# Adttil/crypto12381

Measured on AMD Instinct MI355X. Metric: G1 scalar-muls/s per MI355X (batch 2^20 per GPU), bit-exact vs CPU, higher is better.
Workload: dtype int64 accumulate over 14x28-bit signed limbs

## Files before the change

crypto12381_amd/csrc/g1.hpp:

```cpp
#pragma once
#include "fp.hpp"

namespace c12381 {

struct g1p { fp x, y, z; };

C12381_HD void g1_set_inf(g1p& p) { fp_zero(p.x); fp_one(p.y); fp_zero(p.z); }
C12381_HD bool g1_is_inf(const g1p& p) { return fp_is_zero(p.z); }
C12381_HD void g1_norm1(g1p& r, const g1p& p) { fp_norm1(r.x, p.x); fp_norm1(r.y, p.y); fp_norm1(r.z, p.z); }
C12381_HD void g1_norm1(g1p& p) { g1_norm1(p, p); }
C12381_HD void g1_select(g1p& r, bool c, const g1p& a, const g1p& b) { fp_select(r.x, c, a.x, b.x); fp_select(r.y, c, a.y, b.y); fp_select(r.z, c, a.z, b.z); }
C12381_HD void g1_set_invalid(g1p& p) { fp_one(p.x); fp_zero(p.y); fp_zero(p.z); }
C12381_HD bool g1_is_invalid(const g1p& p) { return fp_is_zero(p.z) && !fp_is_zero(p.x); }

C12381_HD void g1_dbl(g1p& p) {
    fp t0, t1, t2, z8, u, y3, x3, z3;
    const int32_t cm3 = fp_opaque_const(-3);
    fp_mul(t1, p.y, p.z);
    fp_sqr(t2, p.z);
    fp_mul_small(t2, t2, 12);
    fp_sqr_inj(u, p.y, [&](int i, int64_t& acc) { fp_inj(acc, t2, i, cm3); }, C12381_BV(3 * t2.vb), C12381_BV(3 * t2.lb));
    fp_dbl(t0, t2); fp_add(t0, t0, t2); fp_add(t0, t0, u);
    fp_mul_small(z8, t0, 8);
    fp_add(y3, t0, t2);
// ... 163 lines not shown
    {
        uint64_t bw = 0;
#pragma unroll
        for (int i = 0; i < 5; ++i) {
            const uint64_t t = (uint64_t)k[i] - qd[i] - bw;
            rem[i] = (uint32_t)t;
            bw = (t >> 32) & 1;
        }
    }
#pragma unroll
    for (int round = 0; round < 2; ++round) {
        uint32_t d[5];
        uint64_t bw = 0;
#pragma unroll
        for (int i = 0; i < 5; ++i) {
            const uint64_t t = (uint64_t)rem[i] - (i < 4 ? GLV_X2[i] : 0u) - bw;
            d[i] = (uint32_t)t;
            bw = (t >> 32) & 1;
        }
        const bool ge = bw == 0;
#pragma unroll
        for (int i = 0; i < 5; ++i) rem[i] = ge ? d[i] : rem[i];
        uint64_t c = ge ? 1u : 0u;
#pragma unroll
        for (int i = 0; i < 4; ++i) { c += q[i]; q[i] = (uint32_t)c; c >>= 32; }
    }
#pragma unroll
    for (int i = 0; i < 4; ++i) { k0[i] = rem[i]; k1[i] = q[i]; }
}

C12381_HD void soa_store_fp(int32_t* base, size_t stride, size_t idx, const fp& a) {
#pragma unroll
    for (int i = 0; i < NL; ++i) base[(size_t)i * stride + idx] = a.l[i];
}
C12381_HD void soa_load_fp(fp& a, const int32_t* base, size_t stride, size_t idx) {
#pragma unroll
    for (int i = 0; i < NL; ++i) a.l[i] = base[(size_t)i * stride + idx];
    C12381_BOUNDS(a.lb = 268435456.0 + 8.0; a.vb = 4.0; check_actual(a, "soa_load_fp");)
}
C12381_HD void soa_store_g1(int32_t* base, size_t stride, size_t idx, const g1p& p) {
    soa_store_fp(base, stride, idx, p.x);
    soa_store_fp(base + (size_t)NL * stride, stride, idx, p.y);
    soa_store_fp(base + (size_t)2 * NL * stride, stride, idx, p.z);
}
C12381_HD void soa_load_g1(g1p& p, const int32_t* base, size_t stride, size_t idx) {
    soa_load_fp(p.x, base, stride, idx);
    soa_load_fp(p.y, base + (size_t)NL * stride, stride, idx);
    soa_load_fp(p.z, base + (size_t)2 * NL * stride, stride, idx);
}

constexpr int G1_WIN = 5;
constexpr int G1_TAB = 1 << (G1_WIN - 1);
constexpr int G1_WINDOWS = 26;
constexpr int G1_ENT_DWORDS = 44;
constexpr int G1_TAB_DWORDS = G1_TAB * G1_ENT_DWORDS;
struct alignas(16) q4 { int32_t v[4]; };
struct alignas(8) d2 { int32_t v[2]; };

template <int Q0, int NQ, class P>
C12381_HD void rec_store_q4(P dst, const int32_t* w) {
#pragma unroll
    for (int i = Q0; i < Q0 + NQ; ++i) { q4 t; t.v[0] = w[4 * i]; t.v[1] = w[4 * i + 1]; t.v[2] = w[4 * i + 2]; t.v[3] = w[4 * i + 3]; dst[i] = t; }
}
template <int Q0, int NQ, class P>
C12381_HD void rec_load_q4(int32_t* w, P src) {
#pragma unroll
    for (int i = Q0; i < Q0 + NQ; ++i) { q4 t = src[i]; w[4 * i] = t.v[0]; w[4 * i + 1] = t.v[1]; w[4 * i + 2] = t.v[2]; w[4 * i + 3] = t.v[3]; }
}

constexpr double G1_REC_LB = 268435456.0 + 8.0;
template <bool KEEP_PADS = false>
C12381_HD void tab_store_fields(int32_t* ent, const fp& a, const fp& b, const fp& c) {
    int32_t w[G1_ENT_DWORDS];
#pragma unroll
    for (int i = 0; i < NL; ++i) { w[i] = a.l[i]; w[NL + i] = b.l[i]; w[2 * NL + i] = c.l[i]; }
    w[42] = 0; w[43] = 0;
    rec_store_q4<0, G1_ENT_DWORDS / 4 - (KEEP_PADS ? 1 : 0)>(reinterpret_cast<q4*>(ent), w);
    if (KEEP_PADS) { d2 t; t.v[0] = w[40]; t.v[1] = w[41]; *reinterpret_cast<d2*>(ent + 40) = t; }
}
template <bool KEEP_PADS = false>
C12381_HD void tab_store_rec(int32_t* ent, const fp& a, const fp& b, const fp& c, double vb_cap) {
    (void)vb_cap;
    C12381_BOUNDS(for (const fp* e : {&a, &b, &c}) { if (e->vb > vb_cap) bounds_fail("tab_store_rec value bound", e->vb, vb_cap);
                                                      if (e->lb > G1_REC_LB) bounds_fail("tab_store_rec limb bound", e->lb, G1_REC_LB); })
    tab_store_fields<KEEP_PADS>(ent, a, b, c);
}
template <int Q0, int NQ>
C12381_HD void tab_load_q4(int32_t (&w)[G1_ENT_DWORDS], const int32_t* ent) { rec_load_q4<Q0, NQ>(w, reinterpret_cast<const q4*>(ent)); }
C12381_HD void rec_field(fp& a, const int32_t (&w)[G1_ENT_DWORDS], int off, double vb_cap) {
#pragma unroll
    for (int i = 0; i < NL; ++i) a.l[i] = w[off + i];
    (void)vb_cap;
    C12381_BOUNDS(a.lb = G1_REC_LB; a.vb = vb_cap; check_actual(a, "rec_field");)
}
C12381_HD void tab_load_rec(fp& a, fp& b, fp& c, const int32_t* ent, double vb_cap) {
    int32_t w[G1_ENT_DWORDS];
    tab_load_q4<0, G1_ENT_DWORDS / 4>(w, ent);
    rec_field(a, w, 0, vb_cap); rec_field(b, w, NL, vb_cap); rec_field(c, w, 2 * NL, vb_cap);
}
C12381_HD void tab_store_g1(int32_t* ent, const g1p& p) { tab_store_fields(ent, p.x, p.y, p.z); }
C12381_HD void tab_load_g1(g1p& p, const int32_t* ent) { tab_load_rec(p.x, p.y, p.z, ent, 4.0); }

constexpr uint32_t glv_bias_word5(int i) {
    uint32_t v = 0;
    for (int w = 0; w < 26; ++w) { const int bit = 5 * w + 4; if ((bit >> 5) == i) v |= 1u << (bit & 31); }
    return v;
}
C12381_HD int glv_digit(const uint32_t (&kb)[5], int w) {
    const int bit = 5 * w, word = bit >> 5, sh = bit & 31;
    uint32_t v = kb[word] >> sh;
    if (sh > 27) v |= kb[word + 1] << (32 - sh);
    return (int)(v & 31u) - 16;
}
C12381_HD void glv_bias(uint32_t (&kb)[5], const uint32_t (&k)[4]) {
    constexpr uint32_t B[5] = {glv_bias_word5(0), glv_bias_word5(1), glv_bias_word5(2), glv_bias_word5(3), glv_bias_word5(4)};
    uint64_t c = 0;
#pragma unroll
    for (int i = 0; i < 4; ++i) { c += (uint64_t)k[i] + B[i]; kb[i] = (uint32_t)c; c >>= 32; }
    kb[4] = (uint32_t)c + B[4];
}
C12381_HD void glv_scalar_digits(uint32_t (&kb0)[5], uint32_t (&kb1)[5], const uint32_t (&kin)[8], bool zero = false) {
    uint32_t k[8], k0[4], k1[4];
#pragma unroll
    for (int i = 0; i < 8; ++i) k[i] = kin[i];
    scalar_mod_r(k);
    scalar_glv_split(k0, k1, k);
#pragma unroll
    for (int i = 0; i < 4; ++i) { k0[i] = zero ? 0u : k0[i]; k1[i] = zero ? 0u : k1[i]; }
    glv_bias(kb0, k0);
    glv_bias(kb1, k1);
}
C12381_HD const int32_t* g1_digit_entry(const int32_t* lane_tab, int d) {
    const int mag = d < 0 ? -d : d;
    return lane_tab + ((mag == 0 ? 1 : mag) - 1) * G1_ENT_DWORDS;
}
C12381_HD void g1_sched_fence() {
#if defined(__HIP_DEVICE_COMPILE__)
    __builtin_amdgcn_sched_barrier(0);
#endif
}
C12381_HD void g1_digit_fix(g1p& r, g1p q, int d, bool endo);
C12381_HD void g1_digit_point(g1p& r, const int32_t* lane_tab, int d, bool endo) {
    g1p q;
    tab_load_g1(q, g1_digit_entry(lane_tab, d));
    g1_digit_fix(r, q, d, endo);
}
C12381_HD void g1_digit_fix(g1p& r, g1p q, int d, bool endo) {
    const int mag = d < 0 ? -d : d;
    fp ny;
    g1p inf;
    fp_neg(ny, q.y);
    fp_select(q.y, d < 0, ny, q.y);
    g1_set_inf(inf);
    g1_select(q, mag == 0, inf, q);
    C12381_BOUNDS(q.x.lb = q.y.lb = q.z.lb = 268435456.0 + 8.0;)
    if (endo) g1_endo_x2(r, q); else r = q;
}
C12381_HD void g1_add_digit(g1p& acc, const int32_t* lane_tab, int d, bool endo) {
    g1p e;
    g1_digit_point(e, lane_tab, d, endo);
    g1_add(acc, e);
}

C12381_HDN void g1_mul_absx(g1p& p) {
    g1p base, acc;
    g1_norm1(base, p);
    acc = base;
#pragma unroll 1
    for (int i = 62; i >= 0; --i) {
        g1_dbl(acc);
        if ((BLS_X_W[i >> 5] >> (i & 31)) & 1u) g1_add(acc, base);
    }
    p = acc;
}
C12381_HDN void g1_glv_small_scalar_term(g1p& acc, const g1p& base) {
    fp beta;
    fp_set_const(beta, FP_BETA_A);
    g1p q, s1, t;
    fp_mul(q.x, base.x, beta); q.y = base.y; q.z = base.z;
    g1_norm1(q, q);
    s1 = q;
    g1_mul_absx(s1); g1_mul_absx(s1);
    g1_norm1(s1, s1);
    fp_mul(t.x, q.x, beta); t.y = q.y; t.z = q.z;
    g1_norm1(t, t);
    {
        g1p u = s1;
        g1_add(u, t);
        if (g1_is_inf(u)) return;
    }
    g1p s2 = s1;
    g1_mul_absx(s2); g1_mul_absx(s2);
    fp_neg(t.y, s1.y); t.x = s1.x; t.z = s1.z;
    g1_norm1(t, t);
    g1_add(s2, t);
    g1_norm1(s2, s2);
    g1_add(s2, q);
    g1_norm1(s2, s2);
    g1_norm1(acc, acc);
    g1_add(acc, s2);
}

C12381_HDN void g1_scalar_mul_complete(g1p& acc, const fp& px, const fp& py, bool p_is_inf, const uint32_t (&kin)[8], int32_t* lane_tab) {
    uint32_t kb0[5], kb1[5];
    glv_scalar_digits(kb0, kb1, kin);

    g1p base, t;
    base.x = px; base.y = py; fp_one(base.z);
    {
        g1p inf;
        g1_set_inf(inf);
        g1_select(base, p_is_inf, inf, base);
    }
    tab_store_g1(lane_tab, base);
    t = base;
    g1_dbl(t);
    g1_norm1(t);
    tab_store_g1(lane_tab + G1_ENT_DWORDS, t);
#pragma unroll 1
    for (int j = 3; j <= G1_TAB; ++j) {
        if ((j & 1) == 0) {
            tab_load_g1(t, lane_tab + (j / 2 - 1) * G1_ENT_DWORDS);
            g1_dbl(t);
        } else {
            g1_add(t, base);
        }
        g1_norm1(t);
        tab_store_g1(lane_tab + (j - 1) * G1_ENT_DWORDS, t);
    }

    g1_digit_point(acc, lane_tab, glv_digit(kb0, G1_WINDOWS - 1), false);
    g1_norm1(acc);
    g1_add_digit(acc, lane_tab, glv_digit(kb1, G1_WINDOWS - 1), true);
#pragma unroll 1
    for (int w = G1_WINDOWS - 2; w >= 0; --w) {
        const int d0 = glv_digit(kb0, w), d1 = glv_digit(kb1, w);
        g1p q0, q1, e;
        tab_load_g1(q0, g1_digit_entry(lane_tab, d0));
        g1_sched_fence();
#pragma unroll 1
        for (int j = 0; j < G1_WIN; ++j) g1_dbl(acc);
        tab_load_g1(q1, g1_digit_entry(lane_tab, d1));
        g1_sched_fence();
        g1_digit_fix(e, q0, d0, false);
        g1_add(acc, e);
        g1_digit_fix(e, q1, d1, true);
        g1_add(acc, e);
    }
}

C12381_HD void tab_load_xy(fp& x, fp& y, const int32_t* ent) {
    int32_t w[G1_ENT_DWORDS];
    tab_load_q4<0, 7>(w, ent);
    rec_field(x, w, 0, 4.0); rec_field(y, w, NL, 4.0);
}
C12381_HD void tab_load_ybx(fp& y, fp& bx, const int32_t* ent) {
    int32_t w[G1_ENT_DWORDS];
    tab_load_q4<3, 8>(w, ent);
    rec_field(y, w, NL, 4.0); rec_field(bx, w, 2 * NL, 4.0);
}
C12381_HD void tab_fetch_xy(fp& x, fp& y, const int32_t* lane_tab, int d) { tab_load_xy(x, y, g1_digit_entry(lane_tab, d)); g1_sched_fence(); }
C12381_HD void tab_fetch_ybx(fp& y, fp& bx, const int32_t* lane_tab, int d) { tab_load_ybx(y, bx, g1_digit_entry(lane_tab, d)); g1_sched_fence(); }
C12381_HD void tab_store_zt(int32_t* lane_tab, const fp& zt) {
#pragma unroll
    for (int j = 0; j < NL / 2; ++j) { d2 t; t.v[0] = zt.l[2 * j]; t.v[1] = zt.l[2 * j + 1]; *reinterpret_cast<d2*>(lane_tab + j * G1_ENT_DWORDS + 42) = t; }
}
C12381_HD void tab_load_zt(fp& zt, const int32_t* lane_tab) {
#pragma unroll
    for (int j = 0; j < NL / 2; ++j) { const d2 t = *reinterpret_cast<const d2*>(lane_tab + j * G1_ENT_DWORDS + 42); zt.l[2 * j] = t.v[0]; zt.l[2 * j + 1] = t.v[1]; }
    C12381_BOUNDS(zt.lb = G1_REC_LB; zt.vb = 4.0; check_actual(zt, "tab_load_zt");)
}

template <class OnH>
C12381_HD void g1_coz_forward(int32_t* lane_tab, const fp& px, const fp& py, const fp& beta, const OnH& on_h) {
    fp x1, y1, xj, yj, xn, yn, h, hn, bx;
    g1j_dblu(xj, yj, x1, y1, px, py);
#pragma unroll 1
    for (int j = 2; j < G1_TAB; ++j) {
        g1j_zaddu(xn, yn, x1, y1, h, xj, yj);
        fp_norm1(hn, h);
        tab_store_rec(lane_tab + (j - 1) * G1_ENT_DWORDS, xj, yj, hn, 32.0);
        on_h(j, hn);
        xj = xn; yj = yn;
    }
    fp_mul(bx, xj, beta);
    tab_store_rec(lane_tab + (G1_TAB - 1) * G1_ENT_DWORDS, xj, yj, bx, 4.0);
    fp_mul(bx, x1, beta);
    tab_store_rec(lane_tab, x1, y1, bx, 4.0);
}
template <bool KEEP_PADS>
C12381_HD void g1_coz_backward(int32_t* ent, fp& mu, bool first, const fp& beta) {
    fp m2, m3, x, y, h, bx;
    tab_load_rec(x, y, h, ent, 32.0);
    if (first) mu = h; else fp_mul(mu, mu, h);
    fp_sqr(m2, mu);
    fp_mul(m3, m2, mu);
    fp_mul(x, x, m2);
    fp_mul(y, y, m3);
    fp_mul(bx, x, beta);
    tab_store_rec<KEEP_PADS>(ent, x, y, bx, 4.0);
}
C12381_HD void g1j_dbl_window(g1j& a) { g1j_dbl(a); g1j_dbl(a); g1j_dbl(a); g1j_dbl(a); g1j_dbl(a); }

C12381_HD void g1j_add_digit(g1j& acc, bool& acc_inf, const fp& x, const fp& y, int d, bool endo) {
    fp ny, ys, one;
    fp_neg(ny, y);
    fp_select(ys, (d < 0) != endo, ny, y);
    g1j r;
    g1j_madd(r, acc, x, ys);
    fp_one(one);
    fp_select(r.x, acc_inf, x, r.x); fp_select(r.y, acc_inf, ys, r.y); fp_select(r.z, acc_inf, one, r.z);
    const bool keep = d == 0;
    fp_select(acc.x, keep, acc.x, r.x); fp_select(acc.y, keep, acc.y, r.y); fp_select(acc.z, keep, acc.z, r.z);
    acc_inf = acc_inf && keep;
}
C12381_HD bool g1_coz_finish(g1p& acc, const g1j& a, const fp& zc, bool inf) {
    fp z, z2;
    fp_mul(z, a.z, zc);
    const bool exc = !inf && fp_is_zero(z);
    fp_sqr(z2, z);
    fp_mul(acc.x, a.x, z);
    acc.y = a.y;
    fp_mul(acc.z, z2, z);
    g1p o;
    g1_set_inf(o);
    g1_select(acc, inf, o, acc);
    return exc;
}

C12381_HD bool g1_scalar_mul(g1p& acc, const fp& px, const fp& py, bool p_is_inf, const uint32_t (&kin)[8], int32_t* lane_tab) {
    uint32_t kb0[5], kb1[5];
    glv_scalar_digits(kb0, kb1, kin);

    fp beta;
    fp_set_const(beta, FP_BETA_A);
    g1_coz_forward(lane_tab, px, py, beta, [](int, const fp&) {});
    {
        fp mu, zt, y2;
#pragma unroll 1
        for (int j = G1_TAB - 1; j >= 2; --j) g1_coz_backward<false>(lane_tab + (j - 1) * G1_ENT_DWORDS, mu, j == G1_TAB - 1, beta);
        fp_raw_dbl(y2, py);
        fp_mul(zt, mu, y2);
        tab_store_zt(lane_tab, zt);
    }

    g1j a;
    bool acc_inf;
    {
        const int d0 = glv_digit(kb0, G1_WINDOWS - 1);
        fp x, y, ny;
        tab_load_xy(x, y, g1_digit_entry(lane_tab, d0));
        fp_neg(ny, y);
        a.x = x;
        fp_select(a.y, d0 < 0, ny, y);
        fp_one(a.z);
        acc_inf = d0 == 0;
        const int d1 = glv_digit(kb1, G1_WINDOWS - 1);
        tab_load_ybx(y, x, g1_digit_entry(lane_tab, d1));
        g1j_add_digit(a, acc_inf, x, y, d1, true);
    }
#pragma unroll 1
    for (int w = G1_WINDOWS - 2; w >= 0; --w) {
        const int d0 = glv_digit(kb0, w), d1 = glv_digit(kb1, w);
        fp x0, y0, x1, y1;
        tab_fetch_xy(x0, y0, lane_tab, d0);
        g1j_dbl_window(a);
        tab_fetch_ybx(y1, x1, lane_tab, d1);
        g1j_add_digit(a, acc_inf, x0, y0, d0, false);
        g1j_add_digit(a, acc_inf, x1, y1, d1, true);
    }

    fp zt;
    tab_load_zt(zt, lane_tab);
    const bool exc = g1_coz_finish(acc, a, zt, acc_inf || p_is_inf);
    if (exc) g1_scalar_mul_complete(acc, px, py, p_is_inf, kin, lane_tab);
    return exc;
}
C12381_HD void tab_store_kb(int32_t* lane_tab, const uint32_t (&kb0)[5], const uint32_t (&kb1)[5]) {
#pragma unroll
    for (int j = 0; j < 5; ++j) { d2 t; t.v[0] = (int32_t)kb0[j]; t.v[1] = (int32_t)kb1[j]; *reinterpret_cast<d2*>(lane_tab + (NL / 2 + j) * G1_ENT_DWORDS + 42) = t; }
}
C12381_HD void tab_load_kb(uint32_t (&kb0)[5], uint32_t (&kb1)[5], const int32_t* lane_tab) {
#pragma unroll
    for (int j = 0; j < 5; ++j) { const d2 t = *reinterpret_cast<const d2*>(lane_tab + (NL / 2 + j) * G1_ENT_DWORDS + 42); kb0[j] = (uint32_t)t.v[0]; kb1[j] = (uint32_t)t.v[1]; }
}

template <int K, class In>
C12381_HD bool g1_scalar_mul_sum(g1p& acc, const In& in, int32_t* lane_tab) {
    static_assert(K >= 1 && K <= 4, "terms per lane");
    fp beta;
    fp_set_const(beta, FP_BETA_A);
#pragma unroll 1
    for (int t = 0; t < K; ++t) {
        int32_t* tab = lane_tab + t * G1_TAB_DWORDS;
        fp px, py;
        bool p_is_inf;
        uint32_t k[8], kb0[5], kb1[5];
        in(t, px, py, p_is_inf, k);
        glv_scalar_digits(kb0, kb1, k, p_is_inf);
        fp zrun, zt, y2, one;
        g1_coz_forward(tab, px, py, beta, [&](int j, const fp& hn) { if (j == 2) zrun = hn; else fp_mul(zrun, zrun, hn); });
        fp_raw_dbl(y2, py);
        fp_mul(zt, zrun, y2);
        fp_one(one);
        fp_select(zt, p_is_inf, one, zt);
        tab_store_zt(tab, zt);
        tab_store_kb(tab, kb0, kb1);
    }
#pragma unroll 1
    for (int t = 0; t < K; ++t) {
        int32_t* tab = lane_tab + t * G1_TAB_DWORDS;
        fp mu;
        if (K > 1) {
            fp m2, m3, x, y, h, bx;
            bool first = true;
#pragma unroll 1
            for (int l = 0; l < K; ++l) {
                if (l == t) continue;
                tab_load_zt(h, lane_tab + l * G1_TAB_DWORDS);
                if (first) mu = h; else fp_mul(mu, mu, h);
                first = false;
            }
            fp_sqr(m2, mu);
            fp_mul(m3, m2, mu);
#pragma unroll 1
            for (int e = 0; e < 2; ++e) {
                int32_t* ent = tab + (e == 0 ? 0 : G1_TAB - 1) * G1_ENT_DWORDS;
                tab_load_rec(x, y, bx, ent, 4.0);
                fp_mul(x, x, m2);
                fp_mul(y, y, m3);
                fp_mul(bx, bx, m2);
                tab_store_rec<true>(ent, x, y, bx, 4.0);
            }
        }
#pragma unroll 1
        for (int j = G1_TAB - 1; j >= 2; --j) g1_coz_backward<true>(tab + (j - 1) * G1_ENT_DWORDS, mu, K == 1 && j == G1_TAB - 1, beta);
    }

    uint32_t kb[2 * K][5];
#pragma unroll
    for (int t = 0; t < K; ++t) tab_load_kb(kb[2 * t], kb[2 * t + 1], lane_tab + t * G1_TAB_DWORDS);
    g1j a;
    fp_one(a.x); a.y = a.x; a.z = a.x;
    bool acc_inf = true;
#pragma unroll 1
    for (int w = G1_WINDOWS - 1; w >= 0; --w) {
        fp x0, y0, x1, y1;
        int d0 = glv_digit(kb[0], w);
        tab_fetch_xy(x0, y0, lane_tab, d0);
        if (w < G1_WINDOWS - 1) g1j_dbl_window(a);
        const int32_t* tab = lane_tab;
#pragma unroll 1
        for (int t = 0; t < K; ++t) {
            const int d1 = glv_digit(kb[1], w);
            tab_fetch_ybx(y1, x1, tab, d1);
            g1j_add_digit(a, acc_inf, x0, y0, d0, false);
            if (K > 1) {
#pragma unroll
                for (int i = 0; i < 5; ++i) {
                    const uint32_t r0 = kb[0][i], r1 = kb[1][i];
#pragma unroll
                    for (int j = 0; j + 2 < 2 * K; ++j) kb[j][i] = kb[j + 2][i];
                    kb[2 * K - 2][i] = r0; kb[2 * K - 1][i] = r1;
                }
                tab += G1_TAB_DWORDS;
                if (t + 1 < K) {
                    d0 = glv_digit(kb[0], w);
                    tab_fetch_xy(x0, y0, tab, d0);
                }
            }
            g1j_add_digit(a, acc_inf, x1, y1, d1, true);
        }
    }

    fp zc, z;
    tab_load_zt(zc, lane_tab);
#pragma unroll 1
    for (int t = 1; t < K; ++t) {
        tab_load_zt(z, lane_tab + t * G1_TAB_DWORDS);
        fp_mul(zc, zc, z);
    }
    const bool exc = g1_coz_finish(acc, a, zc, acc_inf);
    if (exc) {
#pragma unroll 1
        for (int t = 0; t < K; ++t) {
            fp px, py;
            bool p_is_inf;
            uint32_t k[8];
            in(t, px, py, p_is_inf, k);
            g1p term, n;
            g1_scalar_mul_complete(term, px, py, p_is_inf, k, lane_tab);
            g1_norm1(n, term);
            if (t == 0) { acc = n; continue; }
            g1_add(acc, n);
            g1_norm1(acc);
        }
    }
    return exc;
}
C12381_HD bool scalar_below_x2(const uint32_t (&kin)[8]) {
    uint32_t k[8];
#pragma unroll
    for (int i = 0; i < 8; ++i) k[i] = kin[i];
    scalar_mod_r(k);
    uint64_t bw = 0;
#pragma unroll
    for (int i = 0; i < 4; ++i) { uint64_t t = (uint64_t)k[i] - GLV_X2[i] - bw; bw = (t >> 32) & 1; }
    return (k[4] | k[5] | k[6] | k[7]) == 0u && bw == 1;
}

C12381_HD void g1_to_affine(fp& ax, fp& ay, const g1p& p, const fp& zinv) {
    fp_mul(ax, p.x, zinv);
    fp_mul(ay, p.y, zinv);
}

C12381_HD bool g1_set_x(fp& y, const fp& x, int s) {
    fp x2, x3, four, rhs, c, cinv, ny;
    fp_sqr(x2, x); fp_mul(x3, x2, x);
    fp_set_const(four, FP_FOUR);
    fp_add(rhs, x3, four);
    const bool qr = fp_sqrt_progen(c, cinv, rhs);
    fp_neg(ny, c);
    fp_select(y, fp_sign(c) != s, ny, c);
    return qr;
}

}
```

crypto12381_amd/csrc/k_g1.hip:

```cpp
#include "kernels_common.hpp"
#include "msm.hpp"

using namespace c12381;

namespace c12381 {

__global__ void __launch_bounds__(BLOCK, 2) fp_op_kernel(int op, size_t n, const uint8_t* a, const uint8_t* b, uint8_t* out) {
    const size_t i = (size_t)blockIdx.x * BLOCK + threadIdx.x;
    if (i >= n) return;
    uint32_t raw[12];
    fp x, y, r;
    load_raw48(raw, a + 48 * i); fp_from_raw48(x, raw);
    if (b) { load_raw48(raw, b + 48 * i); fp_from_raw48(y, raw); } else { fp_zero(y); }
    switch (op) {
        case 0: fp_mul(r, x, y); break;
        case 1: fp_add(r, x, y); break;
        case 2: fp_sub(r, x, y); break;
        case 3: fp_sqr(r, x); break;
        case 4: fp_neg(r, x); break;
        default: fp_inv(r, x); break;
    }
    fp_to_raw48(raw, r);
    store_raw48(out + 48 * i, raw);
}

__global__ void __launch_bounds__(BLOCK, 2) fp_mulchain_kernel(size_t n, int iters, const uint8_t* a, const uint8_t* b, uint8_t* out) {
    const size_t i = (size_t)blockIdx.x * BLOCK + threadIdx.x;
    if (i >= n) return;
    uint32_t raw[12];
    fp x, y;
    load_raw48(raw, a + 48 * i); fp_from_raw48(x, raw);
    load_raw48(raw, b + 48 * i); fp_from_raw48(y, raw);
#pragma unroll 1
    for (int it = 0; it < iters; ++it) {
        fp z;
        fp_mul(z, x, y);
        x = y; y = z;
    }
    fp_to_raw48(raw, y);
    store_raw48(out + 48 * i, raw);
}

__global__ void __launch_bounds__(BLOCK, G1_OCC) g1_mul_kernel(size_t n, const uint8_t* pts, size_t pt_stride, const uint8_t* scalars, int32_t* tab,
                                                       int32_t* proj, size_t proj_stride, size_t proj_off, int* bad_flag, const int32_t* skip_if,
                                                       int small_term) {
    if (skip_if && skip_if[HDR_VALID] != 0) return;
    const size_t i = (size_t)blockIdx.x * BLOCK + threadIdx.x;
    if (i >= n) return;
    fp px, py;
    bool inf, ok;
    g1_parse_any(px, py, inf, ok, pts, pt_stride, i);
    uint32_t raw[8], k[8];
    load_raw32(raw, scalars + 32 * i);
    scalar_from_raw32(k, raw);
    g1p acc;
    g1_scalar_mul(acc, px, py, inf || !ok, k, tab + i * (size_t)G1_TAB_DWORDS);
    if (small_term && ok && !inf && scalar_below_x2(k)) {
        g1p base, nn;
        base.x = px; base.y = py; fp_one(base.z);
        g1_norm1(nn, acc);
        g1_glv_small_scalar_term(nn, base);
        acc = nn;
    }
    if (!ok) {
        *bad_flag = 1;
        g1_set_invalid(acc);
    }
    g1p o;
    g1_norm1(o, acc);
    soa_store_g1(proj, proj_stride, proj_off + i, o);
}

__global__ void __launch_bounds__(BLOCK, 2) g1_add_kernel(size_t n, const uint8_t* a, const uint8_t* b, int32_t* proj, size_t proj_stride,
                                                       int* bad_flag) {
    const size_t i = (size_t)blockIdx.x * BLOCK + threadIdx.x;
    if (i >= n) return;
    g1p p, q;
    bool ia, oa, ib, ob;
    g1_parse96_proj(p, ia, oa, a + 96 * i);
    g1_parse96_proj(q, ib, ob, b + 96 * i);
    g1_add(p, q);
    if (!(oa && ob)) { *bad_flag = 1; g1_set_invalid(p); }
    g1_norm1(p);
    soa_store_g1(proj, proj_stride, i, p);
}

__global__ void __launch_bounds__(BLOCK, 2) g1_finish_kernel(size_t n, const int32_t* proj, size_t stride, int32_t* pref, uint8_t* out,
                                                          int fmt, size_t T) {
    const size_t t = (size_t)blockIdx.x * BLOCK + threadIdx.x;
    if (t >= T || t >= n) return;
    const int32_t* zbase = proj + (size_t)2 * NL * stride;
    fp run;
    fp_one(run);
    size_t last = t;
#pragma unroll 1
    for (size_t e = t; e < n; e += T) {
        fp z, one;
        soa_load_fp(z, zbase, stride, e);
        fp_one(one);
        const bool inf = fp_is_zero(z);
        fp_select(z, inf, one, z);
        fp_mul(run, run, z);
        soa_store_fp(pref, stride, e, run);
        last = e;
    }
    fp inv;
    fp_inv(inv, run);
#pragma unroll 1
    for (size_t e = last;; e -= T) {
        g1p p;
        soa_load_g1(p, proj, stride, e);
        fp one, prev, zinv;
        fp_one(one);
        const bool inf = fp_is_zero(p.z), invalid = g1_is_invalid(p);
        fp_select(p.z, inf, one, p.z);
        if (e >= T + t) soa_load_fp(prev, pref, stride, e - T); else prev = one;
        fp_mul(zinv, inv, prev);
        fp_mul(inv, inv, p.z);
        fp ax, ay;
        g1_to_affine(ax, ay, p, zinv);
        uint32_t rx[12], ry[12];
        fp_to_raw48(rx, ax);
        uint8_t* o = out + (size_t)fmt * e;
        if (fmt == 96) {
            fp_to_raw48(ry, ay);
            if (inf) {
#pragma unroll
                for (int j = 0; j < 12; ++j) { rx[j] = invalid ? 0xffffffffu : 0u; ry[j] = invalid ? 0xffffffffu : 0u; }
            }
            store_raw48(o, rx); store_raw48(o + 48, ry);
        } else {
            uint8_t tag = (uint8_t)(0x02 | fp_sign(ay));
            if (inf) {
                tag = invalid ? 0xff : 0x00;
#pragma unroll
                for (int j = 0; j < 12; ++j) rx[j] = invalid ? 0xffffffffu : 0u;
            }
            o[0] = tag;
#pragma unroll
            for (int j = 0; j < 12; ++j) {
                const uint32_t v = rx[j];
                o[1 + 4 * j] = (uint8_t)v; o[2 + 4 * j] = (uint8_t)(v >> 8); o[3 + 4 * j] = (uint8_t)(v >> 16); o[4 + 4 * j] = (uint8_t)(v >> 24);
            }
        }
        if (e < T + t) break;
    }
}

__global__ void __launch_bounds__(BLOCK, 2) g1_reduce_kernel(size_t n, const int32_t* in, size_t in_stride, size_t m, int32_t* outp,
                                                          size_t out_stride) {
    const size_t j = (size_t)blockIdx.x * BLOCK + threadIdx.x;
    if (j >= m) return;
    g1p acc;
    g1_set_inf(acc);
#pragma unroll 1
    for (size_t i = j; i < n; i += m) {
        g1p q;
        soa_load_g1(q, in, in_stride, i);
        g1_add(acc, q);
        g1_norm1(acc);
    }
    soa_store_g1(outp, out_stride, j, acc);
}

__global__ void __launch_bounds__(BLOCK, 2) g1_lift_kernel(size_t n, const uint8_t* pts, int32_t* proj, size_t stride, int* bad_flag) {
    const size_t i = (size_t)blockIdx.x * BLOCK + threadIdx.x;
    if (i >= n) return;
    g1p p, o;
    bool inf, ok;
    g1_parse96_proj(p, inf, ok, pts + 96 * i);
    if (!ok) { *bad_flag = 1; g1_set_inf(p); }
    g1_norm1(o, p);
    soa_store_g1(proj, stride, i, o);
}

__global__ void __launch_bounds__(BLOCK, 2) g1_mul_plain_kernel(size_t n, const uint8_t* pts, const uint8_t* scalars, int32_t* proj, size_t proj_stride, int* bad_flag) {
    const size_t i = (size_t)blockIdx.x * BLOCK + threadIdx.x;
    if (i >= n) return;
    g1p base, acc, inf_pt;
    bool inf, ok;
    g1_parse96_proj(base, inf, ok, pts + 96 * i);
    g1_set_inf(inf_pt);
    if (!ok) base = inf_pt;
    uint32_t raw[8], k[8];
    load_raw32(raw, scalars + 32 * i);
    scalar_from_raw32(k, raw);
    scalar_mod_r(k);
    acc = inf_pt;
#pragma unroll 1
    for (int b = 254; b >= 0; --b) {
        g1_dbl(acc);
        g1p nn, q;
        g1_norm1(nn, acc);
        const bool bit = ((k[b >> 5] >> (b & 31)) & 1u) != 0;
        g1_select(q, bit, base, inf_pt);
        g1_add(nn, q);
        g1_norm1(acc, nn);
    }
    if (!ok) { *bad_flag = 1; g1_set_invalid(acc); }
    soa_store_g1(proj, proj_stride, i, acc);
}

__global__ void __launch_bounds__(BLOCK, 2) g1_add_const_kernel(size_t n, int32_t* proj, size_t stride, const uint8_t* pt96, int* bad_flag) {
    const size_t i = (size_t)blockIdx.x * BLOCK + threadIdx.x;
    if (i >= n) return;
    g1p q, acc;
    bool inf, ok;
    g1_parse96_proj(q, inf, ok, pt96);
    if (!ok) *bad_flag = 1;
    soa_load_g1(acc, proj, stride, i);
    g1_add(acc, q);
    g1p o;
    g1_norm1(o, acc);
    soa_store_g1(proj, stride, i, o);
}

__global__ void __launch_bounds__(BLOCK, 2) g1_rsub_kernel(size_t n, int32_t* acc, size_t acc_stride, const int32_t* other, size_t other_stride,
                                                        size_t other_off, const int32_t* run_if) {
    if (run_if[HDR_VALID] == 0) return;
    const size_t i = (size_t)blockIdx.x * BLOCK + threadIdx.x;
    if (i >= n) return;
    g1p a, b, o;
    soa_load_g1(a, acc, acc_stride, i);
    soa_load_g1(b, other, other_stride, other_off + i);
    fp ny;
    fp_neg(ny, a.y);
    fp_norm1(a.y, ny);
    g1_add(b, a);
    g1_norm1(o, b);
    soa_store_g1(acc, acc_stride, i, o);
}

template <class K>
static __device__ __forceinline__ void msm_prep_body(size_t n, const uint8_t* pts, int in_fmt, const uint8_t* scalars, int c, int W, int32_t* pts2,
                                                     K* keys, uint32_t* vals, int* bad_flag) {
    const size_t i = (size_t)blockIdx.x * BLOCK + threadIdx.x;
    if (i >= n) return;
    uint32_t rp[24], rs[8];
    if (in_fmt == 49) {
        fp x, y; bool inf, ok;
        g1_parse49(x, y, inf, ok, pts + 49 * i);
        if (inf || !ok) { for (int j = 0; j < 24; ++j) rp[j] = 0; if (!ok) rp[23] = 0x01000000u; }
        else { fp_to_raw48(rp, x); fp_to_raw48(rp + 12, y); }
    } else { load_raw48(rp, pts + 96 * i); load_raw48(rp + 12, pts + 96 * i + 48); }
    load_raw32(rs, scalars + 32 * i);
    if (!msm_prep_one<K>(i, n, rp, rs, c, W, pts2, keys, vals)) *bad_flag = 1;
}
__global__ void __launch_bounds__(BLOCK, 2) msm_prep_kernel(size_t n, const uint8_t* pts, int in_fmt, const uint8_t* scalars, int c, int W, int32_t* pts2,
                                                         uint32_t* keys, uint32_t* vals, int* bad_flag) {
    msm_prep_body<uint32_t>(n, pts, in_fmt, scalars, c, W, pts2, keys, vals, bad_flag);
}
__global__ void __launch_bounds__(BLOCK, 2) msm_prep16_kernel(size_t n, const uint8_t* pts, int in_fmt, const uint8_t* scalars, int c, int W, int32_t* pts2,
                                                           uint16_t* keys, int* bad_flag) {
    msm_prep_body<uint16_t>(n, pts, in_fmt, scalars, c, W, pts2, keys, nullptr, bad_flag);
}
__global__ void __launch_bounds__(BLOCK, 2) msm_ranges_kernel(size_t E, const uint32_t* keys, int c, int W, uint32_t* lo, uint32_t* hi) {
    const size_t j = (size_t)blockIdx.x * BLOCK + threadIdx.x;
    if (j >= E) return;
    msm_ranges_one(j, E, keys, c, W, lo, hi);
}
__global__ void __launch_bounds__(BLOCK, 2) msm_ranges16_kernel(size_t n, const uint16_t* keys, int c, int W, uint32_t* lo, uint32_t* hi) {
    constexpr int T = MSM_RANGES_PER_THREAD;
    const uint32_t w = blockIdx.y;
    const uint32_t len = (uint32_t)(w < (uint32_t)W ? 2 * n : n);
    const uint32_t x0 = (blockIdx.x * BLOCK + threadIdx.x) * (uint32_t)T;
    if (x0 >= len) return;
    const size_t seg = (size_t)2 * w * n;
    uint32_t k[T + 2];
#pragma unroll
    for (int j = 0; j < T + 2; ++j) {
        const uint32_t x = x0 + (uint32_t)j;
        k[j] = (x >= 1 && x - 1 < len) ? (uint32_t)keys[seg + x - 1] : 0x10000u;
    }
#pragma unroll
    for (int j = 0; j < T; ++j) {
        const uint32_t x = x0 + (uint32_t)j, d = k[j + 1];
        if (x >= len || d == 0) continue;
        const uint32_t b = w < (uint32_t)W ? ((w << c) | d) : ((uint32_t)W << c);
        if (k[j] != d) lo[b] = (uint32_t)(seg + x);
        if (k[j + 2] != d) hi[b] = (uint32_t)(seg + x + 1);
    }
}
__global__ void __launch_bounds__(BLOCK, 2) msm_sizes_kernel(size_t nbk, const uint32_t* lo, const uint32_t* hi, uint32_t* key, uint32_t* ident,
                                                          uint32_t cap, uint32_t* cnt, uint2* seg, uint4* big, uint32_t early_max) {
    const size_t b = (size_t)blockIdx.x * BLOCK + threadIdx.x;
    if (b >= nbk) return;
    uint32_t len = hi[b] - lo[b];
    if (b == nbk - 1 && len <= early_max) len = 0;
    key[b] = cap - (len < cap ? len : cap);
    ident[b] = (uint32_t)b;
    if (len > cap) {
        const uint32_t sl = cap / 2, ns = (len - cap + sl - 1) / sl;
        const uint32_t base = atomicAdd(&cnt[0], ns);
        const uint32_t q = atomicAdd(&cnt[1], 1u);
        big[q] = make_uint4((uint32_t)b, base, ns, 0u);
        for (uint32_t s = 0; s < ns; ++s) seg[base + s] = make_uint2((uint32_t)b, s);
    }
}
__global__ void __launch_bounds__(BLOCK, MSM_OCC) msm_bucket_kernel(size_t nbk, const uint32_t* lo, const uint32_t* hi, const uint32_t* vals,
                                                           const int32_t* pts2, int32_t* bk, const uint32_t* order, uint32_t cap, uint32_t early_max) {
    const size_t slot = (size_t)blockIdx.x * BLOCK + threadIdx.x;
    if (slot >= nbk) return;
    const size_t b = order[slot];
    g1p acc;
    const size_t l = lo[b];
    size_t h = hi[b];
    if (b == nbk - 1 && h - l <= early_max) h = l;
    msm_bucket_one(acc, l, h - l > cap ? l + cap : h, vals, pts2);
    g1_norm1(acc);
    tab_store_g1(bk + b * G1_ENT_DWORDS, acc);
}
__global__ void __launch_bounds__(BLOCK, 2) msm_overflow_kernel(const uint32_t* cnt, const uint2* seg, const uint32_t* lo, const uint32_t* hi,
                                                             const uint32_t* vals, const int32_t* pts2, int32_t* part, uint32_t cap) {
    const size_t q = (size_t)blockIdx.x * BLOCK + threadIdx.x;
    const uint32_t lane = threadIdx.x & 63u;
    const uint32_t total = cnt[0];
    if (q - lane >= total) return;
    const bool valid = q < total;
    uint32_t bucket = 0xffffffffu;
    g1p acc, t, cand;
    g1_set_inf(acc);
    if (valid) {
        const uint2 e = seg[q];
        bucket = e.x;
        const size_t sl = cap / 2, start = (size_t)lo[e.x] + cap + (size_t)e.y * sl, h = hi[e.x];
        msm_bucket_one(acc, start, h - start > sl ? start + sl : h, vals, pts2);
    }
    g1_norm1(acc);
#pragma unroll 1
    for (int off = 1; off < 64; off <<= 1) {
        const uint32_t ob = (uint32_t)__shfl_down((int)bucket, off, 64);
        g1_shfl_down(t, acc, off);
        cand = acc;
        g1_add(cand, t);
        g1_norm1(cand);
        const bool take = lane + (uint32_t)off < 64u && ob == bucket;
        g1_select(acc, take, cand, acc);
    }
    const uint32_t left = (uint32_t)__shfl_up((int)bucket, 1, 64);
    if (valid && (lane == 0 || left != bucket)) tab_store_g1(part + q * G1_ENT_DWORDS, acc);
}
__global__ void __launch_bounds__(BLOCK, 2) msm_overflow_combine_kernel(const uint32_t* cnt, const uint4* big, const int32_t* part, int32_t* bk) {
    const uint32_t lane = threadIdx.x & 63u;
    const size_t wave = ((size_t)blockIdx.x * BLOCK + threadIdx.x) >> 6, nwaves = ((size_t)gridDim.x * BLOCK) >> 6;
    const uint32_t nbig = cnt[1];
#pragma unroll 1
    for (size_t q = wave; q < nbig; q += nwaves) {
        const uint4 e = big[q];
        const uint32_t base = e.y, end = e.y + e.z, first = (base / 64u + 1u) * 64u;
        const uint32_t heads = 1u + (end > first ? (end - 1u - first) / 64u + 1u : 0u);
        g1p acc, t;
        g1_set_inf(acc);
#pragma unroll 1
        for (uint32_t j0 = 0; j0 < heads; j0 += 64) {
            const uint32_t j = j0 + lane;
            if (j < heads) {
                const uint32_t pos = j == 0 ? base : first + 64u * (j - 1u);
                tab_load_g1(t, part + (size_t)pos * G1_ENT_DWORDS);
                g1_add(acc, t);
// ... 193 lines not shown
```

Baseline: 46.54 million.

## Use Eisenstein-integer joint recoding for G1 scalar multiplication

Replaces the two-scalar GLV windowed ladder with a joint Eisenstein-integer (Z[omega]) recoding. The two GLV halves become a single digit stream of 44 base-8 digits, each taken from an 11-entry table of representatives times the six units. Each window now costs three doublings and a single mixed addition, instead of five doublings and two additions. The trade-offs are a more complex table build with an extra beta^2 field per entry, a longer serial recoding loop, and reliance on the class table covering every residue mod 8 correctly to stay bit-exact.

```diff
diff --git a/crypto12381_amd/csrc/g1.hpp b/crypto12381_amd/csrc/g1.hpp
--- a/crypto12381_amd/csrc/g1.hpp
+++ b/crypto12381_amd/csrc/g1.hpp
@@ -489,15 +489,18 @@
 }
 C12381_HD void g1j_dbl_window(g1j& a) { g1j_dbl(a); g1j_dbl(a); g1j_dbl(a); g1j_dbl(a); g1j_dbl(a); }
 
+C12381_HD void g1j_add_signed(g1j& acc, bool& acc_inf, const fp& x, const fp& y, bool neg, bool keep);
 C12381_HD void g1j_add_digit(g1j& acc, bool& acc_inf, const fp& x, const fp& y, int d, bool endo) {
+    g1j_add_signed(acc, acc_inf, x, y, (d < 0) != endo, d == 0);
+}
+C12381_HD void g1j_add_signed(g1j& acc, bool& acc_inf, const fp& x, const fp& y, bool neg, bool keep) {
     fp ny, ys, one;
     fp_neg(ny, y);
-    fp_select(ys, (d < 0) != endo, ny, y);
+    fp_select(ys, neg, ny, y);
     g1j r;
     g1j_madd(r, acc, x, ys);
     fp_one(one);
     fp_select(r.x, acc_inf, x, r.x); fp_select(r.y, acc_inf, ys, r.y); fp_select(r.z, acc_inf, one, r.z);
-    const bool keep = d == 0;
     fp_select(acc.x, keep, acc.x, r.x); fp_select(acc.y, keep, acc.y, r.y); fp_select(acc.z, keep, acc.z, r.z);
     acc_inf = acc_inf && keep;
 }
@@ -559,6 +562,220 @@
 
     fp zt;
     tab_load_zt(zt, lane_tab);
+    const bool exc = g1_coz_finish(acc, a, zt, acc_inf || p_is_inf);
+    if (exc) g1_scalar_mul_complete(acc, px, py, p_is_inf, kin, lane_tab);
+    return exc;
+}
+constexpr int G1E_TAB = 11;
+constexpr int G1E_DIGITS = 44;
+constexpr uint32_t G1E_NONE = 15;
+constexpr int EIS_REPS[G1E_TAB][2] = {{1, 0}, {2, -1}, {2, -2}, {2, -3}, {1, -3}, {0, -3}, {1, -4}, {2, -4}, {3, -5}, {3, -4}, {4, -4}};
+struct eis_z { int a, b; };
+constexpr eis_z eis_mul_unit(eis_z z, int u) {
+    for (int i = 0; i < u; ++i) z = eis_z{-z.b, z.a + z.b};
+    return z;
+}
+constexpr int eis_chain_unit(int i) {
+    for (int u = 0; u < 6; ++u) {
+        const eis_z w = eis_mul_unit(eis_z{1, 0}, u);
+        if (EIS_REPS[i + 1][0] - EIS_REPS[i][0] == w.a && EIS_REPS[i + 1][1] - EIS_REPS[i][1] == w.b) return u;
+    }
+    return -1;
+}
+constexpr uint32_t eis_chain_deltas() {
+    uint32_t v = 0;
+    int prev = 0;
+    for (int i = 0; i + 1 < G1E_TAB; ++i) {
+        const int u = eis_chain_unit(i);
+        v |= (uint32_t)((u - prev + 6) % 6) << (3 * i);
+        prev = u;
+    }
+    return v;
+}
+constexpr bool eis_chain_ok() {
+    for (int i = 0; i + 1 < G1E_TAB; ++i) if (eis_chain_unit(i) < 0) return false;
+    return eis_chain_unit(G1E_TAB - 2) == 0;
+}
+static_assert(eis_chain_ok(), "the representatives are not a chain of unit steps that ends on +P");
+constexpr uint32_t EIS_CHAIN_DELTAS = eis_chain_deltas();
+struct eis_classes { uint16_t v[64]; };
+constexpr eis_classes eis_make_classes() {
+    eis_classes t{};
+    for (int c = 0; c < 64; ++c) t.v[c] = 0xffff;
+    t.v[0] = (uint16_t)G1E_NONE;
+    for (int e = 0; e < G1E_TAB; ++e)
+        for (int u = 0; u < 6; ++u) {
+            const eis_z d = eis_mul_unit(eis_z{EIS_REPS[e][0], EIS_REPS[e][1]}, u);
+            const int c = (d.a & 7) + 8 * (d.b & 7);
+            if (t.v[c] == 0xffff && d.a >= -5 && d.a <= 5 && d.b >= -5 && d.b <= 5)
+                t.v[c] = (uint16_t)(e | (u << 4) | ((d.a < 0 ? 1 : 0) << 7) | ((d.b < 0 ? 1 : 0) << 8));
+        }
+    return t;
+}
+constexpr bool eis_classes_ok(const eis_classes& t) {
+    for (int c = 0; c < 64; ++c) if (t.v[c] == 0xffff) return false;
+    return true;
+}
+C12381_CONST eis_classes EIS_CLASSES = eis_make_classes();
+static_assert(eis_classes_ok(eis_make_classes()), "a class mod 8 without a representative");
+
+C12381_HD void eis_next(uint32_t (&c)[4], uint32_t t) {
+    uint64_t s = t;
+#pragma unroll
+    for (int i = 0; i < 4; ++i) { s += (c[i] >> 3) | (i < 3 ? c[i + 1] << 29 : 0u); c[i] = (uint32_t)s; s >>= 32; }
+}
+C12381_HD void eis_recode(uint32_t (&kd)[10], const uint32_t (&k0)[4], const uint32_t (&k1)[4]) {
+    uint32_t a[4], b[4];
+#pragma unroll
+    for (int i = 0; i < 4; ++i) { a[i] = k0[i]; b[i] = k1[i]; }
+#pragma unroll
+    for (int i = 0; i < 10; ++i) kd[i] = 0;
+#pragma unroll
+    for (int n = 0; n < G1E_DIGITS; ++n) {
+        const uint32_t e = EIS_CLASSES.v[(a[0] & 7u) | ((b[0] & 7u) << 3)];
+        const int pos = 7 * (G1E_DIGITS - 1 - n), word = pos >> 5, sh = pos & 31;
+        kd[word] |= (e & 127u) << sh;
+        if (sh > 25) kd[word + 1] |= (e & 127u) >> (32 - sh);
+        eis_next(a, (e >> 7) & 1u);
+        eis_next(b, (e >> 8) & 1u);
+    }
+}
+C12381_HD void eis_scalar_digits(uint32_t (&kd)[10], const uint32_t (&kin)[8]) {
+    uint32_t k[8], k0[4], k1[4];
+#pragma unroll
+    for (int i = 0; i < 8; ++i) k[i] = kin[i];
+    scalar_mod_r(k);
+    scalar_glv_split(k0, k1, k);
+    eis_recode(kd, k0, k1);
+}
+C12381_HD uint32_t eis_pop_digit(uint32_t (&kd)[10]) {
+    const uint32_t d = kd[0] & 127u;
+#pragma unroll
+    for (int i = 0; i < 10; ++i) kd[i] = (kd[i] >> 7) | (i < 9 ? kd[i + 1] << 25 : 0u);
+    return d;
+}
+
+constexpr int G1E_FIELD = 16;
+constexpr int G1E_ENT_DWORDS = 4 * G1E_FIELD;
+static_assert(G1E_TAB * G1E_ENT_DWORDS == G1_TAB_DWORDS, "the Eisenstein table fills the lane's record of the 16-entry table");
+C12381_HD void eis_store_field(int32_t* ent, int f, const fp& a, double vb_cap) {
+    (void)vb_cap;
+    C12381_BOUNDS(if (a.vb > vb_cap) bounds_fail("eis_store_field value bound", a.vb, vb_cap);
+                  if (a.lb > G1_REC_LB) bounds_fail("eis_store_field limb bound", a.lb, G1_REC_LB);)
+    int32_t w[G1E_FIELD];
+#pragma unroll
+    for (int i = 0; i < NL; ++i) w[i] = a.l[i];
+    w[14] = 0; w[15] = 0;
+    rec_store_q4<0, G1E_FIELD / 4>(reinterpret_cast<q4*>(ent + f * G1E_FIELD), w);
+}
+C12381_HD void eis_load_field(fp& a, const int32_t* ent, int f, double vb_cap) {
+    int32_t w[G1E_FIELD];
+    rec_load_q4<0, G1E_FIELD / 4>(w, reinterpret_cast<const q4*>(ent + f * G1E_FIELD));
+#pragma unroll
+    for (int i = 0; i < NL; ++i) a.l[i] = w[i];
+    (void)vb_cap;
+    C12381_BOUNDS(a.lb = G1_REC_LB; a.vb = vb_cap; check_actual(a, "eis_load_field");)
+}
+C12381_HD void eis_store_zt(int32_t* lane_tab, const fp& zt) {
+#pragma unroll
+    for (int j = 0; j < NL / 2; ++j) { d2 t; t.v[0] = zt.l[2 * j]; t.v[1] = zt.l[2 * j + 1]; *reinterpret_cast<d2*>(lane_tab + j * G1E_ENT_DWORDS + NL) = t; }
+}
+C12381_HD void eis_load_zt(fp& zt, const int32_t* lane_tab) {
+#pragma unroll
+    for (int j = 0; j < NL / 2; ++j) { const d2 t = *reinterpret_cast<const d2*>(lane_tab + j * G1E_ENT_DWORDS + NL); zt.l[2 * j] = t.v[0]; zt.l[2 * j + 1] = t.v[1]; }
+    C12381_BOUNDS(zt.lb = G1_REC_LB; zt.vb = 4.0; check_actual(zt, "eis_load_zt");)
+}
+C12381_HD void eis_fetch(fp& x, fp& y, const int32_t* lane_tab, uint32_t code) {
+    const uint32_t e = code & 15u, u = code >> 4;
+    const int32_t* ent = lane_tab + (e >= (uint32_t)G1E_TAB ? 0u : e) * G1E_ENT_DWORDS;
+    eis_load_field(y, ent, 0, 4.0);
+    eis_load_field(x, ent, 1 + (int)(u >= 3u ? u - 3u : u), 4.0);
+    g1_sched_fence();
+}
+C12381_HD void g1j_add_eis(g1j& acc, bool& acc_inf, const fp& x, const fp& y, uint32_t code) {
+    g1j_add_signed(acc, acc_inf, x, y, ((code >> 4) & 1u) != 0u, (code & 15u) == G1E_NONE);
+}
+
+C12381_HD void g1e_forward(int32_t* lane_tab, const fp& px, const fp& py, const fp& beta, const fp& beta2) {
+    fp x1 = px, y1 = py, xj = px, yj = py, xn, yn, h, hn, bx;
+#pragma unroll 1
+    for (int i = 0; i + 1 < G1E_TAB; ++i) {
+        const uint32_t dl = (EIS_CHAIN_DELTAS >> (3 * i)) & 7u, m = dl >= 3u ? dl - 3u : dl;
+        if (m != 0u) {
+            fp bm;
+            fp_select(bm, m == 2u, beta2, beta);
+            fp_mul(x1, x1, bm);
+        }
+        if (dl & 1u) fp_neg(y1, y1);
+        g1j_zaddu(xn, yn, x1, y1, h, xj, yj);
+        fp_norm1(hn, h);
+        int32_t* ent = lane_tab + i * G1E_ENT_DWORDS;
+        eis_store_field(ent, 0, yj, 32.0); eis_store_field(ent, 1, xj, 32.0); eis_store_field(ent, 2, hn, 32.0);
+        xj = xn; yj = yn;
+    }
+    int32_t* last = lane_tab + (G1E_TAB - 1) * G1E_ENT_DWORDS;
+    eis_store_field(last, 0, yj, 4.0); eis_store_field(last, 1, xj, 4.0);
+    fp_mul(bx, xj, beta); eis_store_field(last, 2, bx, 4.0);
+    fp_mul(bx, xj, beta2); eis_store_field(last, 3, bx, 4.0);
+    eis_store_field(lane_tab, 0, y1, 4.0); eis_store_field(lane_tab, 1, x1, 4.0);
+    fp_mul(bx, x1, beta2); eis_store_field(lane_tab, 3, bx, 4.0);
+}
+C12381_HD void g1e_backward(int32_t* ent, fp& mu, bool first, const fp& beta, const fp& beta2) {
+    fp m2, m3, x, y, h, bx;
+    eis_load_field(y, ent, 0, 32.0); eis_load_field(x, ent, 1, 32.0); eis_load_field(h, ent, 2, 32.0);
+    if (first) mu = h; else fp_mul(mu, mu, h);
+    fp_sqr(m2, mu);
+    fp_mul(m3, m2, mu);
+    fp_mul(x, x, m2);
+    fp_mul(y, y, m3);
+    eis_store_field(ent, 0, y, 4.0); eis_store_field(ent, 1, x, 4.0);
+    fp_mul(bx, x, beta); eis_store_field(ent, 2, bx, 4.0);
+    fp_mul(bx, x, beta2); eis_store_field(ent, 3, bx, 4.0);
+}
+
+C12381_HD bool g1_scalar_mul_eis(g1p& acc, const fp& px, const fp& py, bool p_is_inf, const uint32_t (&kin)[8], int32_t* lane_tab) {
+    uint32_t kd[10];
+    eis_scalar_digits(kd, kin);
+
+    fp beta, beta2;
+    fp_set_const(beta, FP_BETA_A);
+    fp_set_const(beta2, FP_BETA_B);
+    g1e_forward(lane_tab, px, py, beta, beta2);
+    {
+        fp mu, zt, h0, x, bx;
+#pragma unroll 1
+        for (int i = G1E_TAB - 2; i >= 1; --i) g1e_backward(lane_tab + i * G1E_ENT_DWORDS, mu, i == G1E_TAB - 2, beta, beta2);
+        eis_load_field(h0, lane_tab, 2, 32.0);
+        eis_load_field(x, lane_tab, 1, 4.0);
+        fp_mul(zt, mu, h0);
+        fp_mul(bx, x, beta);
+        eis_store_field(lane_tab, 2, bx, 4.0);
+        eis_store_zt(lane_tab, zt);
+    }
+
+    g1j a;
+    bool acc_inf;
+    {
+        const uint32_t code = eis_pop_digit(kd);
+        fp x, y, ny;
+        eis_fetch(x, y, lane_tab, code);
+        fp_neg(ny, y);
+        a.x = x;
+        fp_select(a.y, ((code >> 4) & 1u) != 0u, ny, y);
+        fp_one(a.z);
+        acc_inf = (code & 15u) == G1E_NONE;
+    }
+#pragma unroll 1
+    for (int w = G1E_DIGITS - 2; w >= 0; --w) {
+        const uint32_t code = eis_pop_digit(kd);
+        fp x, y;
+        eis_fetch(x, y, lane_tab, code);
+        g1j_dbl(a); g1j_dbl(a); g1j_dbl(a);
+        g1j_add_eis(a, acc_inf, x, y, code);
+    }
+
+    fp zt;
+    eis_load_zt(zt, lane_tab);
     const bool exc = g1_coz_finish(acc, a, zt, acc_inf || p_is_inf);
     if (exc) g1_scalar_mul_complete(acc, px, py, p_is_inf, kin, lane_tab);
     return exc;
diff --git a/crypto12381_amd/csrc/k_g1.hip b/crypto12381_amd/csrc/k_g1.hip
--- a/crypto12381_amd/csrc/k_g1.hip
+++ b/crypto12381_amd/csrc/k_g1.hip
@@ -54,7 +54,7 @@
     load_raw32(raw, scalars + 32 * i);
     scalar_from_raw32(k, raw);
     g1p acc;
-    g1_scalar_mul(acc, px, py, inf || !ok, k, tab + i * (size_t)G1_TAB_DWORDS);
+    g1_scalar_mul_eis(acc, px, py, inf || !ok, k, tab + i * (size_t)G1_TAB_DWORDS);
     if (small_term && ok && !inf && scalar_below_x2(k)) {
         g1p base, nn;
         base.x = px; base.y = py; fp_one(base.z);
```

After: 50.78 million, median of 6. +9.1%, better.
